# gwenzhang/GGA

Measured on AMD Instinct MI355X. Metric: kitti_frames_per_sec_gga_train_step, higher is better.
Workload: dtype f32 tensors; products on 2 x f16 operand planes (block-scaled), f32 accumulate - measured no less accurate than fp32 kernels: per convolution 0.7 x (dense) / 0.7-1.2 x (sparse) the RMS error of an fp32 FMA chain vs float64, whole-step losses over 8 seeds <= 2.5e-5 from float64 (fp32 CPU step: <= 1.6

## Files before the change

gga_amd/_lib.py:

```python
import ctypes as C
import os
import subprocess

_HERE = os.path.dirname(os.path.abspath(__file__))
LIB_PATH = os.path.join(_HERE, 'libgga_hip.so')
ABI_VERSION = 31

_lib = None

vp, i32, i64, f32, sz = C.c_void_p, C.c_int, C.c_int64, C.c_float, C.c_size_t
I3 = C.POINTER(C.c_int32 * 3)


class VoxelParams(C.Structure):
    _fields_ = [('voxel_size', C.c_float * 3), ('pc_range', C.c_float * 6),
                ('max_points', C.c_int32), ('max_voxels', C.c_int32)]


class PfnParams(C.Structure):
    _fields_ = [('voxel_size', C.c_float * 3), ('offsets', C.c_float * 3), ('eps', C.c_float),
                ('momentum', C.c_float), ('training', C.c_int32), ('in_features', C.c_int32),
                ('channels', C.c_int32)]


MAX_TASKS = 8


class Task(C.Structure):
    _fields_ = [('logits', vp), ('target', vp), ('n_heat', i64), ('focal_out', vp), ('focal_grad', vp), ('grad_logits', vp),
# ... 76 lines not shown
    'gga_dense_conv3x3_levels': (i32, [i32, vp, vp, vp, vp, i32, i32, i32, vp, i64, i32, vp, vp, vp, i32, i32, vp, vp]),
    'gga_dense_conv3x3_bn_bwd_pays': (i32, [i32, i32, i32, i32]),
    'gga_dense_conv3x3_bn_bwd_pays_planes': (i32, [i32, i32, i32, i32, i32]),
    'gga_dense_conv3x3_bn_bwd': (i32, [vp, vp, i32, i32, i32, i32, i32, vp, i64, i32, vp, i32, vp, vp, vp, i64, vp, vp, vp, vp, vp]),
    'gga_absmax_table_blocks': (i64, [i64]),
    'gga_absmax_table': (i32, [vp, i32, i64, vp, i32, vp]),
    'gga_pack_weights_table': (i32, [vp, i32, i64, i32, vp]),
    'gga_dense_wgrad3x3_block_amax': (i32, [vp, vp, i32, i32, i32, i32, i32, vp, i64, i64, i64, i64, i32, i32, vp, i32, vp, i32, vp, sz, vp]),
    'gga_dense_conv3x3_tile_rows': (i32, [i32, i32, i32, i32, i32]),
    'gga_dense_conv3x3_stat_rows': (i64, [i32, i32, i32, i32, i32, i32]),
    'gga_bn_stats_partials': (i32, [vp, vp, vp, vp, i64, i32, f32, f32, vp, vp, vp, i32, vp]),
    'gga_bn_stats_partials_cols': (i32, [vp, vp, vp, vp, i64, i32, f32, f32, vp, vp, vp, i32, i32, i32, vp]),
    'gga_bn_relu_workspace_bytes': (sz, [i64, i32]),
    'gga_bn_relu_mask_bytes': (sz, [i64, i32]),
    'gga_bn_relu_fwd_ex': (i32, [vp, vp, vp, vp, vp, vp, i64, i32, f32, f32, i32, i32, vp, i64, vp, vp, vp, i32, vp, vp, sz, vp]),
    'gga_bn_relu_bwd_ex': (i32, [vp, i64, vp, vp, vp, vp, i64, i32, i32, i32, vp, vp, vp, vp, vp, vp, sz, vp]),
    'gga_column_sums': (i32, [vp, i64, i32, vp, vp, sz, vp]),
    'gga_bn_relu_bwd_partials': (i32, [vp, i64, vp, vp, vp, i64, i32, i32, vp, i32, vp, vp, vp, vp, vp, sz, vp]),
    'gga_gn_relu_workspace_bytes': (sz, [i32, i32]),
    'gga_gn_relu_fwd': (i32, [vp, vp, vp, i32, i64, i32, i32, f32, i32, vp, vp, vp, vp, vp, sz, vp]),
    'gga_gn_relu_bwd': (i32, [vp, vp, vp, vp, vp, i32, i64, i32, i32, i32, vp, vp, vp, vp, vp, sz, vp]),
    'gga_bn_stats': (i32, [vp, vp, vp, vp, vp, i64, i32, f32, f32, i32, vp, vp, vp, sz, vp]),
    'gga_head_conv3x3_fwd': (i32, [vp, i64, vp, vp, vp, i32, i32, i32, i32, i32, vp, vp]),
    'gga_head_conv3x3_workspace_bytes': (sz, [i32]),
    'gga_head_conv3x3_wgrad': (i32, [vp, i64, vp, vp, i32, i32, i32, i32, i32, vp, vp, vp, sz, vp]),
    'gga_head_tail_bwd': (i32, [vp, vp, i64, vp, vp, vp, vp, i32, i32, i32, i32, i32, vp, i64, vp, vp, vp, vp, sz, vp]),
    'gga_head_tile_activity': (i32, [vp, i32, i32, i32, i32, vp, vp]),
    'gga_head_branch_bwd_workspace_bytes': (sz, [i32, i32, i32, i32]),
    'gga_head_branch_bwd': (i32, [vp, vp, i64, vp, vp, vp, vp, i32, i32, i32, i32, i32, vp, vp, vp, i64, vp, vp, vp, i32, vp, sz, vp]),
    'gga_heatmap_splat': (i32, [vp, i32, i32, i32, vp, i32, vp, vp, i32, vp]),
    'gga_focal_loss_workspace_bytes': (sz, [i64, i32]),
    'gga_focal_loss_fwd': (i32, [C.POINTER(TaskTable), f32, f32, f32, vp, sz, vp]),
    'gga_focal_loss_bwd': (i32, [C.POINTER(TaskTable), f32, f32, f32, vp]),
    'gga_gather_pred_fwd': (i32, [C.POINTER(TaskTable), i32, i32, i32, i32, vp]),
    'gga_gather_pred_bwd': (i32, [C.POINTER(TaskTable), i32, i32, i32, i32, vp]),
    'gga_box_losses_workspace_bytes': (sz, [i32, i32, i32]),
    'gga_box_losses_fwd': (i32, [C.POINTER(TaskTable), C.POINTER(LossParams), vp, sz, vp]),
    'gga_box_losses_bwd': (i32, [C.POINTER(TaskTable), i32, i32, vp]),
    'gga_box_iou_rotated': (i32, [vp, i32, vp, i32, i32, i32, vp, vp]),
    'gga_nms_rotated_workspace_bytes': (sz, [i32]),
    'gga_nms_rotated_sorted': (i32, [vp, i32, f32, i32, vp, vp, vp, sz, vp]),
    'gga_circle_nms_sorted': (i32, [vp, i32, C.c_double, i32, vp, vp, vp, sz, vp]),
    'gga_region_grow_workspace_bytes': (sz, [i64, i32]),
    'gga_region_grow': (i32, [vp, i64, i32, vp, vp, vp, i32, C.c_double, i32, vp, vp, sz, vp]),
    'gga_points_in_convex_polyhedra': (i32, [vp, i64, i32, vp, vp, i32, i32, vp, vp]),
    'gga_plane_inliers': (i32, [vp, i64, i32, vp, i32, C.c_double, vp, vp, vp]),
# ... 68 lines not shown
```

gga_amd/csrc/api.cc:

```cpp
#include <hip/hip_runtime.h>
#include <stdarg.h>
#include <stdio.h>

#include <mutex>
#include <vector>

#include "../../include/gga_hip.h"

static thread_local char g_err[512] = "";

void gga_set_error(const char* fmt, ...) {
    va_list ap;
    va_start(ap, fmt);
    vsnprintf(g_err, sizeof(g_err), fmt, ap);
    va_end(ap);
}

extern "C" const char* gga_last_error(void) { return g_err; }
extern "C" int gga_abi_version(void) { return 31; }

struct TimingSite {
    std::vector<hipEvent_t> ev;
    int cap = 0, count = 0;
    int64_t key = 0;
};
static TimingSite g_sites[GGA_TIME_SITES];
static std::mutex g_timing_mu;

hipEvent_t* gga_timing_acquire(int site, int64_t key) {
    if (site < 0 || site >= GGA_TIME_SITES) return nullptr;
    TimingSite& s = g_sites[site];
    if (s.cap == 0) return nullptr;
    std::lock_guard<std::mutex> lk(g_timing_mu);
    if (s.count >= s.cap || (s.key != 0 && s.key != key)) return nullptr;
    return &s.ev[2 * (size_t)s.count++];
}

extern "C" int gga_timing_begin(int site, int max_samples, int64_t key) {
    if (site < 0 || site >= GGA_TIME_SITES || max_samples < 0 || max_samples > 65536) {
        gga_set_error("gga_timing_begin: site %d / max_samples %d out of range", site, max_samples);
        return GGA_ERR_INVALID_ARG;
    }
// ... 36 lines not shown
```

gga_amd/csrc/headconv.hip:

```cpp
#include "gga_common.h"

#define HC_CIN 64
#define HC_MAXCO 4

#define HM_TW 32
#define HM_HW (HM_TW + 2)
#define HP_TR 13
#define HP_HR (HP_TR + 2)
#define HP_NPIX (HP_HR * HM_HW)
#define HP_NGRP 16
static_assert((HP_NPIX + 31) / 32 == HP_NGRP, "tile geometry");

template <int COUT, bool AFF>
__global__ __launch_bounds__(512, 4) void headconv_fwd16_kernel(const float* __restrict__ x, const float* __restrict__ w,
                                                            const float* __restrict__ bias, int B, int H, int W,
                                                            int tiles_x, int tiles_y, int n_tiles, int cout_total, int co_base,
                                                            const float* __restrict__ in_ss, int64_t xs, float* __restrict__ y) {
    typedef float f4 __attribute__((ext_vector_type(4)));
    typedef float f2 __attribute__((ext_vector_type(2)));
    constexpr int NT = COUT == 1 ? 1 : 2;
    constexpr int ZS = (9 * COUT) | 1;
    __shared__ float zt[HP_NGRP * 32 * ZS];
    __shared__ __attribute__((aligned(16))) float wl[16 * NT * 64];
    __shared__ __attribute__((aligned(16))) float ssl[4 * HC_CIN];
    __shared__ float bl[HC_MAXCO];
    const int per_img = tiles_x * tiles_y;
    const int lane = threadIdx.x & 63, wave = threadIdx.x >> 6;
    const int n = lane & 15, hq = lane >> 4;
    for (int i = threadIdx.x; i < 16 * NT * 64; i += 512) {
        const int e = i & 3, nn = (i >> 2) & 15, t = (i >> 6) % NT, jh = i / (64 * NT);
        const int c = 16 * (jh >> 2) + 4 * (jh & 3) + e, col = 16 * t + nn;
        const bool used = col < 9 * COUT;
        const int off = used ? col / COUT : 0, co = used ? col - off * COUT : 0;
        wl[i] = used ? w[((int64_t)(co_base + co) * HC_CIN + c) * 9 + off] : 0.0f;
    }
    if (AFF && threadIdx.x < 4 * HC_CIN) ssl[threadIdx.x] = threadIdx.x < 2 * HC_CIN ? in_ss[threadIdx.x] : 0.0f;
    if (threadIdx.x < COUT) bl[threadIdx.x] = bias ? bias[co_base + threadIdx.x] : 0.0f;
    __syncthreads();
    int loff[2][2], hrc[2][2];
#pragma unroll
// ... 36 lines not shown
                    const f2 hi = __builtin_elementwise_fma(f2{v[s][2], v[s][3]}, f2{sc[2], sc[3]}, f2{sf[2], sf[3]}); \
                    v[s] = f4{fmaxf(lo[0], 0.0f), fmaxf(lo[1], 0.0f), fmaxf(hi[0], 0.0f), fmaxf(hi[1], 0.0f)};       \
                }                                                                                                     \
            } else {                                                                                                  \
                _Pragma("unroll") for (int s = 0; s < 2; ++s) {                                                       \
                    const bool ok = (okm[U] >> s) & 1u;                                                               \
                    _Pragma("unroll") for (int e = 0; e < 4; ++e) v[s][e] = ok ? v[s][e] : 0.0f;                      \
                }                                                                                                     \
            }                                                                                                         \
            _Pragma("unroll") for (int e = 0; e < 4; ++e)                                                             \
                _Pragma("unroll") for (int t = 0; t < NT; ++t) {                                                      \
                    HQ_MFMA_(acc[0][t], v[0][e], bc[t][e]) HQ_MFMA_(acc[1][t], v[1][e], bc[t][e])                     \
                }                                                                                                     \
        }                                                                                                             \
        _Pragma("unroll") for (int s = 0; s < 2; ++s) _Pragma("unroll") for (int t = 0; t < NT; ++t)                  \
            if (16 * t + n < 9 * COUT) {                                                                              \
                float* zg = zt + ((wave + 8 * (U)) * 32 + 16 * s + 4 * hq) * ZS + 16 * t + n;                         \
                _Pragma("unroll") for (int v_ = 0; v_ < 4; ++v_) zg[v_ * ZS] = acc[s][t][v_];                         \
            } }
#define HQ_MFMA_(ACC, A, Bv) ACC = __builtin_amdgcn_mfma_f32_16x16x4f32(A, Bv, ACC, 0, 0, 0);
    const int xcd = blockIdx.x & 7, wg = blockIdx.x >> 3, wgs = ((int)gridDim.x + 7 - xcd) >> 3;
    const int chunk = (n_tiles + 7) >> 3;
    const int t_end = min(n_tiles, (xcd + 1) * chunk);
    int tile = xcd * chunk + wg;
    if (tile >= t_end) return;
    HQ_LOAD(tile, true, 0)
    HQ_LOAD(tile, true, 1)
    for (; tile < t_end; tile += wgs) {
        const int b = tile / per_img;
        const int rem = tile - b * per_img;
        const int y0 = (rem / tiles_x) * HP_TR, x0 = (rem % tiles_x) * HM_TW;
        const int nxt = tile + wgs;
        HQ_MMA(0)
        HQ_LOAD(nxt, nxt < t_end, 0)
        HQ_MMA(1)
        HQ_LOAD(nxt, nxt < t_end, 1)
        __syncthreads();
        if (threadIdx.x < HP_TR * HM_TW) {
            const int ty = threadIdx.x / HM_TW, tx = threadIdx.x - ty * HM_TW;
            const int oy = y0 + ty, ox = x0 + tx;
            if (oy < H && ox < W) {
                float s[COUT];
#pragma unroll
                for (int co = 0; co < COUT; ++co) s[co] = bl[co];
#pragma unroll
                for (int ky = 0; ky < 3; ++ky)
#pragma unroll
                    for (int kx = 0; kx < 3; ++kx) {
                        const float* z = zt + ((ty + ky) * HM_HW + tx + kx) * ZS + (ky * 3 + kx) * COUT;
#pragma unroll
                        for (int co = 0; co < COUT; ++co) s[co] += z[co];
                    }
                float* yo = y + (((int64_t)b * cout_total + co_base) * H + oy) * W + ox;
#pragma unroll
                for (int co = 0; co < COUT; ++co) yo[(int64_t)co * H * W] = s[co];
// ... 13 lines not shown
#define HG_PR (HG_TR + 2)
#define HG_PC (HG_TW + 2)
#define HG_GP (HG_PR * HG_PC)

__global__ __launch_bounds__(256) void head_tile_activity_kernel(const float* __restrict__ gy, int cout, int H, int W, int tiles_x,
                                                                 int tiles_y, int64_t n_tiles, uint8_t* __restrict__ act) {
    const int64_t t = (int64_t)blockIdx.x * 4 + (threadIdx.x >> 6);
    if (t >= n_tiles) return;
    const int lane = threadIdx.x & 63;
    const int per_img = tiles_x * tiles_y;
    const int b = (int)(t / per_img), rem = (int)(t - (int64_t)b * per_img);
    const int y0 = (rem / tiles_x) * HG_TR, x0 = (rem % tiles_x) * HG_TW;
    const int ya = max(y0 - 1, 0), yb = min(y0 + HG_TR, H - 1), xa = max(x0 - 1, 0), xb = min(x0 + HG_TW, W - 1);
    const int nc = xb - xa + 1, per_ch = (yb - ya + 1) * nc;
    uint32_t bits = 0;
    for (int i = lane; i < cout * per_ch; i += 64) {
        const int c = i / per_ch, q = i - c * per_ch;
        const int r = q / nc, col = q - r * nc;
        bits |= __float_as_uint(gy[(((int64_t)b * cout + c) * H + ya + r) * W + xa + col]);
    }
    const bool any = __ballot(bits != 0) != 0;
    if (lane == 0) act[t] = any ? 1 : 0;
}

struct HeadTileWalk {
    const uint8_t* act;
    int64_t base, stride, n_tiles;
    unsigned long long mask;
    __device__ __forceinline__ unsigned long long window(int64_t from) const {
        const int64_t t = from + (int64_t)(threadIdx.x & 63) * stride;
        return __ballot(t < n_tiles && act[t] != 0);
    }
    __device__ __forceinline__ HeadTileWalk(const uint8_t* a, int64_t first, int64_t s, int64_t n) : act(a), base(first), stride(s), n_tiles(n) {
        mask = window(base);
    }
    __device__ __forceinline__ int64_t next() {
        while (mask == 0) {
            if (base + 64 * stride >= n_tiles) return n_tiles;
            base += 64 * stride;
            mask = window(base);
        }
        const int k = __builtin_ctzll(mask);
        mask &= mask - 1;
        return base + k * stride;
    }
};

template <int COUT, bool AFF, bool MAP>
__global__ __launch_bounds__(512, 4) void headconv_wgrad16_kernel(const float* __restrict__ x, const float* __restrict__ dy,
                                                              int B, int H, int W, int tiles_x, int tiles_y, int n_tiles,
                                                              int cout_total, int co_base, const float* __restrict__ in_ss,
                                                              int64_t xs, const uint8_t* __restrict__ act,
                                                              float* __restrict__ partials) {
    typedef float f4 __attribute__((ext_vector_type(4)));
    typedef float f2 __attribute__((ext_vector_type(2)));
    constexpr int NT = COUT == 1 ? 1 : 2;
    constexpr int GN = (COUT * HG_GP + 511) / 512;
    __shared__ float gds[2][(COUT + 1) * HG_GP];
    __shared__ float red[HC_CIN * 33];
    __shared__ float bred[GN * 512];
    const int tid = threadIdx.x, lane = tid & 63, wave = tid >> 6;
    const int n = lane & 15, hq = lane >> 4;
    const int per_img = tiles_x * tiles_y;
    int gb[NT];
#pragma unroll
    for (int t = 0; t < NT; ++t) {
        const int col = n + 16 * t;
        const bool used = col < 9 * COUT;
        const int off = used ? col / COUT : 4, co = used ? col - off * COUT : COUT;
// ... 153 lines not shown
                "%s: specialised for %d input channels and 1..%d output channels (got %d -> %d)", fn, HC_CIN, HC_MAXCO,
                cin, cout);
    return GGA_OK;
}

extern "C" size_t gga_head_conv3x3_workspace_bytes(int cout) {
    return (size_t)HC_BLOCKS * ((size_t)cout * HC_CIN * 9 + cout) * sizeof(float);
}

static int headconv_stride(const char* fn, const void* x, int64_t xs) {
    GGA_REQUIRE(xs >= HC_CIN && xs % 4 == 0 && ((uintptr_t)x & 15) == 0,
                "%s: pixel stride %lld must be a multiple of 4 floats >= %d and the base 16-byte aligned", fn, (long long)xs, HC_CIN);
    return GGA_OK;
}

static int headconv_limits(const char* fn, int H, int W, int64_t xs, int rows, int64_t n_tiles) {
    GGA_REQUIRE(H < 16384 && W < 16384, "%s: height and width must be below 16384 (got H=%d W=%d)", fn, H, W);
    GGA_REQUIRE((int64_t)rows * W * xs < 2147483647ll,
                "%s: %d * W * pixel stride must be below 2^31 elements (got W=%d, pixel stride %lld)", fn, rows, W, (long long)xs);
    GGA_REQUIRE(n_tiles < 2147483647ll, "%s: too many tiles (%lld)", fn, (long long)n_tiles);
    return GGA_OK;
}

extern "C" int gga_head_conv3x3_fwd(const float* x, int64_t x_pixel_stride, const float* in_scale_shift, const float* weight,
                                    const float* bias, int B, int H, int W, int cin, int cout, float* y, void* stream_) {
    hipStream_t stream = (hipStream_t)stream_;
    if (int rc = headconv_check("gga_head_conv3x3_fwd", B, H, W, cin, cout)) return rc;
    GGA_REQUIRE(x && weight && y, "gga_head_conv3x3_fwd: null pointer argument");
    if (int rc = headconv_stride("gga_head_conv3x3_fwd", x, x_pixel_stride)) return rc;
    const int tx = (W + HM_TW - 1) / HM_TW, ty = (H + HP_TR - 1) / HP_TR;
    const int64_t n_tiles = (int64_t)B * tx * ty;
    if (int rc = headconv_limits("gga_head_conv3x3_fwd", H, W, x_pixel_stride, HP_HR + 1, n_tiles)) return rc;
    const dim3 grid((unsigned)(n_tiles < HC_BLOCKS ? n_tiles : HC_BLOCKS)), block(512);
#define HC_G(CO, BASE, AF) hipLaunchKernelGGL((headconv_fwd16_kernel<CO, AF>), grid, block, 0, stream, x, weight, bias, B, H, W, tx, ty, (int)n_tiles, cout, BASE, in_scale_shift, x_pixel_stride, y)
#define HC_F(CO, BASE) { if (in_scale_shift) HC_G(CO, BASE, true); else HC_G(CO, BASE, false); }
    switch (cout) {
        case 1: HC_F(1, 0); break;
        case 2: HC_F(2, 0); break;
        case 3: HC_F(3, 0); break;
        default: HC_F(2, 0); HC_F(2, 2); break;
    }
#undef HC_F
#undef HC_G
    GGA_CHECK_LAUNCH("headconv_fwd16_kernel");
    return GGA_OK;
}

static int headconv_wgrad_run(const char* fn, const float* x, int64_t x_pixel_stride, const float* in_scale_shift,
                              const float* grad_y, int B, int H, int W, int cin, int cout, float* grad_weight, float* grad_bias,
                              void* workspace, size_t workspace_bytes, const uint8_t* tile_act, hipStream_t stream) {
    if (int rc = headconv_check(fn, B, H, W, cin, cout)) return rc;
    if (int rc = headconv_stride(fn, x, x_pixel_stride)) return rc;
    GGA_REQUIRE(x && grad_y && grad_weight && workspace, "%s: null pointer argument", fn);
    const int tx = (W + HG_TW - 1) / HG_TW, ty = (H + HG_TR - 1) / HG_TR;
    const int64_t n_tiles = (int64_t)B * tx * ty;
    if (int rc = headconv_limits(fn, H, W, x_pixel_stride, HG_TR, n_tiles)) return rc;
    if (workspace_bytes < gga_head_conv3x3_workspace_bytes(cout)) {
        gga_set_error("%s: workspace too small", fn);
        return GGA_ERR_WORKSPACE;
    }
    const int nb = (int)(n_tiles < HC_BLOCKS ? n_tiles : HC_BLOCKS);
    float* partials = (float*)workspace;
#define HC_G(CO, BASE, AF, MP) hipLaunchKernelGGL((headconv_wgrad16_kernel<CO, AF, MP>), dim3(nb), dim3(512), 0, stream, x, grad_y, B, H, W, tx, ty, (int)n_tiles, cout, BASE, in_scale_shift, x_pixel_stride, tile_act, partials)
#define HC_A(CO, BASE, AF) { if (tile_act) HC_G(CO, BASE, AF, true); else HC_G(CO, BASE, AF, false); }
#define HC_W(CO, BASE) { if (in_scale_shift) HC_A(CO, BASE, true) else HC_A(CO, BASE, false) }
    switch (cout) {
        case 1: HC_W(1, 0); break;
// ... 329 lines not shown
```

gga_amd/dense_heads.py:

```python
import copy

import numpy as np
import os

import torch
from torch import nn

from . import dense_conv
from . import functional as F
from . import ops
from .cnn import ConvModule, build_conv_layer, kaiming_init
from .registry import HEADS, build_bbox_coder, build_head, build_loss

SRL_PRIORS = ((1.35, 0.48), (3.60, 0.68), (2.40, 0.28))


def multi_apply(func, *args, **kwargs):
    from functools import partial
    pfunc = partial(func, **kwargs) if kwargs else func
    return tuple(map(list, zip(*map(pfunc, *args))))


@HEADS.register_module()
class SeparateHead(nn.Module):
    def __init__(self, in_channels, heads, head_conv=64, final_kernel=1, init_bias=-2.19,
                 conv_cfg=dict(type='Conv2d'), norm_cfg=dict(type='BN2d'), bias='auto', init_cfg=None, **kwargs):
        assert init_cfg is None, 'To prevent abnormal initialization behavior, init_cfg is not allowed to be set'
        super().__init__()
        self.heads = heads
        self.init_bias = init_bias
        for head in self.heads:
            classes, num_conv = self.heads[head]
            conv_layers = []
            c_in = in_channels
            for _ in range(num_conv - 1):
                conv_layers.append(ConvModule(c_in, head_conv, kernel_size=final_kernel, stride=1,
                                              padding=final_kernel // 2, bias=bias, conv_cfg=conv_cfg,
# ... 76 lines not shown
        self.bbox_coder = build_bbox_coder(bbox_coder) if bbox_coder is not None else None
        self.num_anchor_per_locs = [n for n in num_classes]
        self.fp16_enabled = False
        self.pal_backprop = pal_backprop

        self.shared_conv = ConvModule(in_channels, share_conv_channel, kernel_size=3, padding=1,
                                      conv_cfg=conv_cfg, norm_cfg=norm_cfg, bias=bias)
        self.task_heads = nn.ModuleList()
        separate_head = dict(separate_head)
        for num_cls in num_classes:
            heads = copy.deepcopy(common_heads)
            heads.update(dict(heatmap=(num_cls, num_heatmap_convs)))
            separate_head.update(in_channels=share_conv_channel, heads=heads, num_cls=num_cls)
            self.task_heads.append(build_head(separate_head))
        self.with_velocity = 'vel' in common_heads.keys()
        assert not self.with_velocity, 'GGA does not support velocity (head:600-601)'
        assert self.norm_bbox, 'the HIP loss path implements norm_bbox=True (log-dims), as every GGA config uses'
        for name in ('loss_cls', 'loss_bbox'):
            red = getattr(getattr(self, name), 'reduction', 'mean')
            if red != 'mean':
                raise NotImplementedError(f"CenterHead_GGA: {name}.reduction={red!r}; the HIP loss path implements "
                                          f"reduction='mean' (configs/gga/gga_kitti_config.py:59-60)")

    def forward_single(self, x):
        x = self.shared_conv(x)
        branches, keys = [], []
        for ti, task in enumerate(self.task_heads):
            for head in getattr(task, 'heads', ()):
                mods = list(getattr(task, head))
                if (isinstance(task, SeparateHead) and len(mods) == 2 and isinstance(mods[0], ConvModule) and mods[0].with_norm
                        and mods[0].with_activation and isinstance(mods[0].norm, nn.modules.batchnorm._BatchNorm)
                        and isinstance(mods[0].activate, nn.ReLU)):
                    branches.append((mods[0].conv, mods[0].norm, mods[1]))
                    keys.append((ti, head))
        n_all = sum(len(getattr(task, 'heads', ())) for task in self.task_heads)
        outs = (F.head_branches(x, branches, sparse_grad=[head != 'heatmap' for _, head in keys])
                if branches and len(branches) == n_all and self.training else None)
        if outs is None:
            return [task(x) for task in self.task_heads]
        ret = [dict() for _ in self.task_heads]
        for (ti, head), y in zip(keys, outs):
            ret[ti][head] = y
        return ret

    def forward(self, feats):
        return multi_apply(self.forward_single, feats)

    def _feature_map_size(self):
        g = self.train_cfg['grid_size']
        osf = self.train_cfg['out_size_factor']
        return int(g[0]) // int(osf), int(g[1]) // int(osf)

    def draw_srl(self, batch_size):
        out = np.zeros((batch_size, len(self.task_heads)), np.float32)
        for b in range(batch_size):
            for t in range(len(self.task_heads)):
                mu, sd = SRL_PRIORS[t] if t < 2 else SRL_PRIORS[2]
                r = torch.normal(torch.tensor(mu), torch.tensor(sd))
                out[b, t] = float(torch.clamp(r, min=1e-3))
        return out

    def pack_targets(self, gt_labels_3d, GGA_boxes_img, GGA_lidar2img, GGA_init_pseudo_labels, GGA_bdry_masks,
                     GGA_in_box_points, img_metas, srl=None):
        tc = self.train_cfg
        B, T = len(gt_labels_3d), len(self.task_heads)
        K = int(tc['max_objs']) * int(tc['dense_reg'])
        osf = tc['out_size_factor']
        fw, fh = self._feature_map_size()
        vs = np.asarray(tc['voxel_size'], np.float32).astype(np.float64)
# ... 290 lines not shown
```

gga_amd/detectors.py:

```python
from collections import OrderedDict

import torch
from torch import nn

from .registry import (DETECTORS, build_backbone, build_head, build_middle_encoder, build_neck,
                       build_voxel_encoder)
from .voxel_layer import Voxelization


def _sub(cfg, key):
    if cfg is None:
        return None
    return cfg[key] if isinstance(cfg, dict) else getattr(cfg, key)


class PreparedInputs:

    def __init__(self, voxels, num_points, coors, n_frames):
        self.voxels, self.num_points, self.coors, self.n_frames = voxels, num_points, coors, n_frames

    def __len__(self):
        return self.n_frames

    def tensors(self):
        yield from (t for t in (self.voxels, self.num_points, self.coors) if t is not None)
        for extra in (getattr(self.coors, 'num_valid', None),):
            if extra is not None:
# ... 104 lines not shown
        if self.dynamic_voxelization:
            if self.front_reads_counts:
                coors.voxel_map.host_counts()
            return PreparedInputs(voxels, None, coors, len(points))
        if hasattr(self.pts_middle_encoder, 'build_indices'):
            coors = self.pts_middle_encoder.build_indices(coors, len(points))
        return PreparedInputs(voxels, num_points, coors, len(points))

    def forward_train(self, points=None, img_metas=None, gt_bboxes_3d=None, gt_labels_3d=None,
                      GGA_boxes_img=None, GGA_lidar2img=None, GGA_init_pseudo_labels=None, GGA_bdry_masks=None,
                      GGA_in_box_points=None, gt_labels=None, gt_bboxes=None, img=None, proposals=None,
                      gt_bboxes_ignore=None):
        img_feats, pts_feats = self.extract_feat(points, img=img, img_metas=img_metas)
        losses = dict()
        if pts_feats:
            losses.update(self.forward_pts_train(pts_feats, gt_bboxes_3d, gt_labels_3d, GGA_boxes_img,
                                                 GGA_lidar2img, GGA_init_pseudo_labels, GGA_bdry_masks,
                                                 GGA_in_box_points, img_metas, gt_bboxes_ignore))
        return losses

    def forward_pts_train(self, pts_feats, gt_bboxes_3d, gt_labels_3d, GGA_boxes_img, GGA_lidar2img,
                          GGA_init_pseudo_labels, GGA_bdry_masks, GGA_in_box_points, img_metas,
                          gt_bboxes_ignore=None):
        outs = self.pts_bbox_head(pts_feats)
        return self.pts_bbox_head.loss(gt_bboxes_3d, gt_labels_3d, outs, GGA_boxes_img, GGA_lidar2img,
                                       GGA_init_pseudo_labels, GGA_bdry_masks, GGA_in_box_points, img_metas)

    def forward(self, return_loss=True, **kwargs):
        if return_loss:
            return self.forward_train(**kwargs)
        return self.forward_test(**kwargs)

    def forward_test(self, points, img_metas, img=None, **kwargs):
        for var, name in [(points, 'points'), (img_metas, 'img_metas')]:
            if not isinstance(var, list):
                raise TypeError(f'{name} must be a list, but got {type(var)}')
        if len(points) != len(img_metas):
            raise ValueError(f'num of augmentations ({len(points)}) != num of image meta ({len(img_metas)})')
        if len(points) == 1:
            return self.simple_test(points[0], img_metas[0], None if img is None else img[0], **kwargs)
        raise NotImplementedError('test-time augmentation is not on the GGA path')

    @torch.no_grad()
    def simple_test_pts(self, x, img_metas, rescale=False):
        from .box3d import bbox3d2result
        outs = self.pts_bbox_head(x)
        bbox_list = self.pts_bbox_head.get_bboxes(outs, img_metas, rescale=rescale)
# ... 45 lines not shown
```

gga_amd/functional.py:

```python
import ctypes as C

import numpy as np
import torch

from . import _lib
from ._lib import LossParams, PfnParams, VoxelParams, check
import contextlib
import os

_DEFERRED_COUNTERS = None


def count_batch(bn):
    if _DEFERRED_COUNTERS is not None:
        _DEFERRED_COUNTERS.append(bn.num_batches_tracked)
    else:
        bn.num_batches_tracked += 1


@contextlib.contextmanager
def deferred_batch_counters():
    global _DEFERRED_COUNTERS
    prev, _DEFERRED_COUNTERS = _DEFERRED_COUNTERS, []
    try:
# ... 965 lines not shown
          and bn.momentum is not None and bn.training and torch.is_grad_enabled() and conv.out_channels <= 4
          and conv.kernel_size == (3, 3) and conv.stride == (1, 1) and conv.padding == (1, 1)
          and conv.dilation == (1, 1) and conv.groups == 1 and conv.padding_mode == 'zeros')
    if not ok:
        return head_conv3x3(bn_act(x, bn, relu=True), conv)
    count_batch(bn)
    partials = bn_partials_of(x)
    return _BnReluHeadConv3x3.apply(x, bn.weight, bn.bias, bn.running_mean, bn.running_var, conv.weight, conv.bias,
                                    float(bn.eps), float(bn.momentum), True, partials, sparse_grad)


_BRANCH_STREAMS = {}
HEAD_STREAMS = int(os.environ.get('GGA_HEAD_STREAMS', '2'))


def _branch_streams(device, n):
    k = max(1, min(HEAD_STREAMS, n))
    pool = _BRANCH_STREAMS.setdefault(device, [])
    while len(pool) < k - 1:
        pool.append(torch.cuda.Stream(device=device))
    return [torch.cuda.current_stream(device)] + pool[:k - 1]


class _HeadBranches(torch.autograd.Function):

    @staticmethod
    def forward(ctx, x, n, cfg, *t):
        from . import dense_conv
        w1, gam, bet, rm, rv, w2, b2 = (t[i * n:(i + 1) * n] for i in range(7))
        L = _lib.lib()
        B, C, H, W = x.shape
        rows, dev, tot = B * H * W, x.device, C * n
        tr = dense_conv._transposed(H, W)
        Y = torch.empty((B, tot, H, W), dtype=torch.float32, device=dev, memory_format=torch.channels_last)
        outs, saved_all, ss_all = [], [], []
        x_amax = dense_conv.tensor_amax(x) if dense_conv.PLANES == 2 else None
        pair_stats = {}
        for i in range(0, n - 1, 2):
            _, st = dense_conv._run(x, [w1[i].detach(), w1[i + 1].detach()], False, True, x_amax, None, Y, C * i)
            pair_stats[i], pair_stats[i + 1] = (st, 0), (st, C)
        all_stats = []
        for i in range(n):
            if i in pair_stats:
                all_stats.append(pair_stats[i])
            else:
                all_stats.append((dense_conv._run(x, w1[i].detach(), False, True, x_amax, None, Y, C * i)[1], 0))
        w2c = [w.contiguous() for w in w2]
        for i in range(n):
            outs.append(torch.empty((B, w2[i].shape[0], H, W), dtype=torch.float32, device=dev))
            saved_all.append(torch.empty(2 * C, dtype=torch.float32, device=dev))
            ss_all.append(torch.empty(2 * C, dtype=torch.float32, device=dev))
        streams = _branch_streams(dev, n)
        for st_ in streams[1:]:
            st_.wait_stream(streams[0])
        for i in range(n):
            eps, momentum = cfg[i][:2]
            stats, col = all_stats[i]
            tiles = int(stats.shape[0])
            with torch.cuda.stream(streams[i % len(streams)]):
                check(L.gga_bn_stats_partials_cols(_p(gam[i]), _p(bet[i]), _p(rm[i]), _p(rv[i]), rows, C, eps, momentum,
                                                   _p(saved_all[i]), _p(ss_all[i]), _p(stats), tiles, int(stats.shape[2]), col,
                                                   _stream()), 'gga_bn_stats_partials_cols')
                check(L.gga_head_conv3x3_fwd(Y.data_ptr() + 4 * C * i, tot, _p(ss_all[i]), _p(w2c[i]), _p(b2[i]), B, H, W, C,
                                             w2[i].shape[0], _p(outs[i]), _stream()), 'gga_head_conv3x3_fwd')
        for st_ in streams[1:]:
            streams[0].wait_stream(st_)
        ctx.save_for_backward(x, Y, *w1, *gam, *w2, *saved_all, *ss_all)
        ctx.n, ctx.has_bias, ctx.x_amax = n, [b is not None for b in b2], x_amax
        ctx.sparse_grad = [int(c[2]) for c in cfg]
        ctx.bn_src = dense_conv.bn_source(x, C) if dense_conv.BN_BWD_FUSED else None
        return tuple(outs)

    @staticmethod
    def backward(ctx, *gys):
        from . import dense_conv
        n = ctx.n
        t = ctx.saved_tensors
        x, Y = t[0], t[1]
        w1, gam, w2, saved_all, ss_all = (t[2 + i * n:2 + (i + 1) * n] for i in range(5))
        L = _lib.lib()
        B, C, H, W = x.shape
        rows, dev, tot = B * H * W, x.device, C * n
        G = torch.empty_like(Y)
        g_blocks = dense_conv.new_amax(dev, n)
        gw2, gb2, ggam, gbet = [], [], [], []
        gyc = [g.contiguous() for g in gys]
        w2c = [w.contiguous() for w in w2]
# ... 1 lines not shown
            gw2.append(torch.empty_like(w2c[i]))
            gb2.append(torch.empty(w2[i].shape[0], dtype=torch.float32, device=dev) if ctx.has_bias[i] else None)
            ggam.append(torch.empty(C, dtype=torch.float32, device=dev))
            gbet.append(torch.empty(C, dtype=torch.float32, device=dev))
        streams = _branch_streams(dev, n)
        for st_ in streams[1:]:
            st_.wait_stream(streams[0])
        for i in range(n):
            cout = w2[i].shape[0]
            with torch.cuda.stream(streams[i % len(streams)]):
                ws = _workspace('headbranch', L.gga_head_branch_bwd_workspace_bytes(B, H, W, cout), dev)
                check(L.gga_head_branch_bwd(_p(gyc[i]), Y.data_ptr() + 4 * C * i, tot, _p(ss_all[i]), _p(gam[i]), _p(saved_all[i]),
                                            _p(w2c[i]), B, H, W, C, cout, _p(gw2[i]), _p(gb2[i]), G.data_ptr() + 4 * C * i, tot,
                                            _p(ggam[i]), _p(gbet[i]), _p(g_blocks[i:i + 1] if g_blocks is not None else None),
                                            ctx.sparse_grad[i], _p(ws), ws.numel(), _stream()), 'gga_head_branch_bwd')
        for st_ in streams[1:]:
            streams[0].wait_stream(st_)
        wcat = [w.detach() for w in w1]
        g_amax = g_blocks.max().reshape(1) if g_blocks is not None else None
        gx = dense_conv.run_bn_bwd(G, wcat, g_amax, None, ctx.bn_src) if ctx.needs_input_grad[0] else None
        gwcat = dense_conv._wgrad(x, G, wcat, ctx.x_amax if dense_conv.PLANES == 2 else None, g_blocks, g_per_block=True)
        gw1 = list(gwcat.split(C, dim=0))
        none = [None] * n
        return (gx, None, None, *gw1, *ggam, *gbet, *none, *none, *gw2, *gb2)


def head_branches(x, branches, sparse_grad=None):
    from . import dense_conv
    rc = _rows_channels(x) if (x.is_cuda and x.dtype == torch.float32 and x.dim() == 4) else None
    if rc is None or x.shape[1] != 64 or not torch.is_grad_enabled() or not dense_conv.ENABLED or not dense_conv.WGRAD:
        return None
    for conv1, bn, conv2 in branches:
        ok = (dense_conv.eligible(conv1, x) and conv1.bias is None and conv1.out_channels == 64 and bn.affine
              and bn.track_running_stats and bn.momentum is not None and bn.training and conv2.out_channels <= 4
              and type(conv2) is torch.nn.Conv2d and conv2.in_channels == 64 and conv2.kernel_size == (3, 3)
              and conv2.stride == (1, 1) and conv2.padding == (1, 1) and conv2.dilation == (1, 1) and conv2.groups == 1
              and conv2.padding_mode == 'zeros')
        if not ok:
            return None
    for _, bn, _ in branches:
        count_batch(bn)
    n = len(branches)
    sparse = [True] * n if sparse_grad is None else [bool(s) for s in sparse_grad]
    assert len(sparse) == n
    cfg = tuple((float(bn.eps), float(bn.momentum), s) for (_, bn, _), s in zip(branches, sparse))
    cols = ([c1.weight for c1, _, _ in branches], [bn.weight for _, bn, _ in branches], [bn.bias for _, bn, _ in branches],
            [bn.running_mean for _, bn, _ in branches], [bn.running_var for _, bn, _ in branches],
            [c2.weight for _, _, c2 in branches], [c2.bias for _, _, c2 in branches])
    return _HeadBranches.apply(x, n, cfg, *[t for col in cols for t in col])


def head_conv3x3(x, conv):
    ok = (x.is_cuda and x.dtype == torch.float32 and x.dim() == 4 and x.shape[1] == 64
          and x.is_contiguous(memory_format=torch.channels_last) and conv.out_channels <= 4
          and conv.kernel_size == (3, 3) and conv.stride == (1, 1) and conv.padding == (1, 1)
          and conv.dilation == (1, 1) and conv.groups == 1 and conv.padding_mode == 'zeros')
    if not ok:
        return conv(x)
    return _HeadConv3x3.apply(x, conv.weight, conv.bias)


def centerpoint_detect(boxes, scores, labels, coder_range, coder_score_threshold, score_threshold, limit_range, nms_threshold,
                       pre_max_size, post_max_size, num_classes):
    _need_cuda(boxes, scores, labels)
    T, B, K, D = boxes.shape
    dev = boxes.device
    boxes, scores, labels = boxes.float().contiguous(), scores.float().contiguous(), labels.float().contiguous()
    out_boxes = torch.empty((B, T * K, D), dtype=torch.float32, device=dev)
    out_scores = torch.empty((B, T * K), dtype=torch.float32, device=dev)
    out_labels = torch.empty((B, T * K), dtype=torch.int32, device=dev)
    count = torch.zeros((B,), dtype=torch.int32, device=dev)
    offs, flag = [], 0
# ... 15 lines not shown
```

include/gga_hip.h:

```cpp
#ifndef GGA_HIP_H_
#define GGA_HIP_H_

#include <stddef.h>
#include <stdint.h>

#ifdef __cplusplus
extern "C" {
#endif

typedef enum {
    GGA_OK = 0,
    GGA_ERR_INVALID_ARG = -1,
    GGA_ERR_WORKSPACE = -2,
    GGA_ERR_LAUNCH = -3
} gga_status;

const char* gga_last_error(void);
int gga_abi_version(void);

enum {
    GGA_TIME_SCATTER_FWD = 0,
    GGA_TIME_DENSE_CONV = 1,
    GGA_TIME_SPARSE_CONV = 2,
    GGA_TIME_SPARSE_WGRAD = 3,
// ... 222 lines not shown
                    void* stream);
int gga_bn_relu_bwd_partials(const float* grad_masked, int64_t grad_row_stride, const float* x, const float* gamma,
                             const float* saved, int64_t rows, int channels, int training, const double* partials,
                             int n_partials, float* grad_x, float* grad_gamma, float* grad_beta, uint32_t* amax_grad_x,
                             void* workspace, size_t workspace_bytes, void* stream);

size_t gga_gn_relu_workspace_bytes(int B, int channels);
int gga_gn_relu_fwd(const float* x, const float* gamma, const float* beta, int B, int64_t rows_per_sample, int channels,
                    int groups, float eps, int relu, float* y, float* stat, float* scale_shift, uint32_t* amax_y,
                    void* workspace, size_t workspace_bytes, void* stream);
int gga_gn_relu_bwd(const float* grad_y, const float* x, const float* gamma, const float* stat, const float* scale_shift,
                    int B, int64_t rows_per_sample, int channels, int groups, int relu, float* grad_x, float* grad_gamma,
                    float* grad_beta, uint32_t* amax_grad_x, void* workspace, size_t workspace_bytes, void* stream);

int gga_bn_stats_partials(const float* gamma, const float* beta, float* running_mean, float* running_var,
                          int64_t rows, int channels, float eps, float momentum, float* saved, float* scale_shift,
                          const double* partials, int n_partials, void* stream);
int gga_bn_stats_partials_cols(const float* gamma, const float* beta, float* running_mean, float* running_var, int64_t rows,
                               int channels, float eps, float momentum, float* saved, float* scale_shift, const double* partials,
                               int n_partials, int partials_width, int column_offset, void* stream);

int gga_head_conv3x3_fwd(const float* x, int64_t x_pixel_stride, const float* in_scale_shift, const float* weight,
                         const float* bias, int B, int H, int W, int cin, int cout, float* y, void* stream);
size_t gga_head_conv3x3_workspace_bytes(int cout);
int gga_head_conv3x3_wgrad(const float* x, int64_t x_pixel_stride, const float* in_scale_shift, const float* grad_y,
                           int B, int H, int W, int cin, int cout, float* grad_weight, float* grad_bias,
                           void* workspace, size_t workspace_bytes, void* stream);

int gga_head_tail_bwd(const float* grad_y, const float* x, int64_t x_pixel_stride, const float* scale_shift,
                      const float* gamma, const float* saved, const float* weight, int B, int H, int W, int cin, int cout,
                      float* grad_x, int64_t grad_x_pixel_stride, float* grad_gamma, float* grad_beta, uint32_t* amax_grad_x,
                      void* workspace, size_t workspace_bytes, void* stream);

int gga_head_tile_activity(const float* grad_y, int B, int H, int W, int cout, uint8_t* tile_active, void* stream);

size_t gga_head_branch_bwd_workspace_bytes(int B, int H, int W, int cout);
int gga_head_branch_bwd(const float* grad_y, const float* x, int64_t x_pixel_stride, const float* scale_shift,
                        const float* gamma, const float* saved, const float* weight, int B, int H, int W, int cin, int cout,
                        float* grad_weight, float* grad_bias, float* grad_x, int64_t grad_x_pixel_stride, float* grad_gamma,
                        float* grad_beta, uint32_t* amax_grad_x, int sparse_grad_y, void* workspace, size_t workspace_bytes,
                        void* stream);

int gga_heatmap_splat(float* heatmap, int n_maps, int H, int W, const int32_t* objs, int n_obj,
                      const float* patch_table, const int32_t* patch_offsets, int max_radius,
                      void* stream);

// ... 149 lines not shown
```

Before: 525.4.

## Compute regression head forward convs only on tiles containing target cells

The training step now builds targets before the head forward and marks which 13x32 output tiles contain any target index for each task. The final 3x3 head conv for non-heatmap branches runs a tile-mapped kernel that skips inactive tiles and leaves zeros there, since only gathered cells feed the regression losses. This removes most of the dense forward conv work for regression branches. In exchange it adds a zero-fill of those outputs and a small marking kernel, and it makes the branch outputs valid only at target cells.

```diff
diff --git a/gga_amd/_lib.py b/gga_amd/_lib.py
--- a/gga_amd/_lib.py
+++ b/gga_amd/_lib.py
@@ -4,7 +4,7 @@
 
 _HERE = os.path.dirname(os.path.abspath(__file__))
 LIB_PATH = os.path.join(_HERE, 'libgga_hip.so')
-ABI_VERSION = 31
+ABI_VERSION = 32
 
 _lib = None
 
@@ -127,6 +127,9 @@
     'gga_gn_relu_bwd': (i32, [vp, vp, vp, vp, vp, i32, i64, i32, i32, i32, vp, vp, vp, vp, vp, sz, vp]),
     'gga_bn_stats': (i32, [vp, vp, vp, vp, vp, i64, i32, f32, f32, i32, vp, vp, vp, sz, vp]),
     'gga_head_conv3x3_fwd': (i32, [vp, i64, vp, vp, vp, i32, i32, i32, i32, i32, vp, vp]),
+    'gga_head_conv3x3_fwd_tiles': (i32, [vp, i64, vp, vp, vp, i32, i32, i32, i32, i32, vp, vp, vp]),
+    'gga_head_cell_tiles_count': (i64, [i32, i32, i32]),
+    'gga_head_cell_tiles': (i32, [vp, i32, i32, i32, i32, vp, vp]),
     'gga_head_conv3x3_workspace_bytes': (sz, [i32]),
     'gga_head_conv3x3_wgrad': (i32, [vp, i64, vp, vp, i32, i32, i32, i32, i32, vp, vp, vp, sz, vp]),
     'gga_head_tail_bwd': (i32, [vp, vp, i64, vp, vp, vp, vp, i32, i32, i32, i32, i32, vp, i64, vp, vp, vp, vp, sz, vp]),
diff --git a/gga_amd/csrc/api.cc b/gga_amd/csrc/api.cc
--- a/gga_amd/csrc/api.cc
+++ b/gga_amd/csrc/api.cc
@@ -17,7 +17,7 @@
 }
 
 extern "C" const char* gga_last_error(void) { return g_err; }
-extern "C" int gga_abi_version(void) { return 31; }
+extern "C" int gga_abi_version(void) { return 32; }
 
 struct TimingSite {
     std::vector<hipEvent_t> ev;
diff --git a/gga_amd/csrc/headconv.hip b/gga_amd/csrc/headconv.hip
--- a/gga_amd/csrc/headconv.hip
+++ b/gga_amd/csrc/headconv.hip
@@ -11,11 +11,51 @@
 #define HP_NGRP 16
 static_assert((HP_NPIX + 31) / 32 == HP_NGRP, "tile geometry");
 
-template <int COUT, bool AFF>
+struct HeadTileWalk {
+    const uint8_t* act;
+    int64_t base, stride, n_tiles;
+    unsigned long long mask;
+    __device__ __forceinline__ unsigned long long window(int64_t from) const {
+        const int64_t t = from + (int64_t)(threadIdx.x & 63) * stride;
+        return __ballot(t < n_tiles && act[t] != 0);
+    }
+    __device__ __forceinline__ HeadTileWalk(const uint8_t* a, int64_t first, int64_t s, int64_t n) : act(a), base(first), stride(s), n_tiles(n) {
+        mask = window(base);
+    }
+    __device__ __forceinline__ int64_t next() {
+        while (mask == 0) {
+            if (base + 64 * stride >= n_tiles) return n_tiles;
+            base += 64 * stride;
+            mask = window(base);
+        }
+        const int k = __builtin_ctzll(mask);
+        mask &= mask - 1;
+        return base + k * stride;
+    }
+};
+
+__global__ __launch_bounds__(256) void head_cell_tiles_kernel(const int64_t* __restrict__ ind, int64_t n, int K, int H, int W,
+                                                              int tiles_x, int tiles_y, uint8_t* __restrict__ act) {
+    const int64_t s = (int64_t)blockIdx.x * 256 + threadIdx.x;
+    if (s >= n) return;
+    const int64_t i = ind[s];
+    if (i < 0 || i >= (int64_t)H * W) return;
+    const int cy = (int)(i / W), cx = (int)(i - (int64_t)cy * W);
+    act[((s / K) * tiles_y + cy / HP_TR) * tiles_x + cx / HM_TW] = 1;
+}
+
+template <int COUT, bool AFF, bool MAP>
 __global__ __launch_bounds__(512, 4) void headconv_fwd16_kernel(const float* __restrict__ x, const float* __restrict__ w,
                                                             const float* __restrict__ bias, int B, int H, int W,
                                                             int tiles_x, int tiles_y, int n_tiles, int cout_total, int co_base,
-                                                            const float* __restrict__ in_ss, int64_t xs, float* __restrict__ y) {
+                                                            const float* __restrict__ in_ss, int64_t xs, float* __restrict__ y,
+                                                            const uint8_t* __restrict__ act) {
+    if (MAP) {
+        const int xcd_ = blockIdx.x & 7, chunk_ = (n_tiles + 7) >> 3;
+        const int end_ = min(n_tiles, (xcd_ + 1) * chunk_);
+        HeadTileWalk probe(act, xcd_ * chunk_ + ((int)blockIdx.x >> 3), ((int)gridDim.x + 7 - xcd_) >> 3, end_);
+        if (probe.next() >= end_) return;
+    }
     typedef float f4 __attribute__((ext_vector_type(4)));
     typedef float f2 __attribute__((ext_vector_type(2)));
     constexpr int NT = COUT == 1 ? 1 : 2;
@@ -98,15 +138,16 @@
     const int xcd = blockIdx.x & 7, wg = blockIdx.x >> 3, wgs = ((int)gridDim.x + 7 - xcd) >> 3;
     const int chunk = (n_tiles + 7) >> 3;
     const int t_end = min(n_tiles, (xcd + 1) * chunk);
-    int tile = xcd * chunk + wg;
+    HeadTileWalk walk(MAP ? act : nullptr, MAP ? xcd * chunk + wg : t_end, wgs, t_end);
+    int tile = MAP ? (int)walk.next() : xcd * chunk + wg;
     if (tile >= t_end) return;
     HQ_LOAD(tile, true, 0)
     HQ_LOAD(tile, true, 1)
-    for (; tile < t_end; tile += wgs) {
+    for (int nxt; tile < t_end; tile = nxt) {
         const int b = tile / per_img;
         const int rem = tile - b * per_img;
         const int y0 = (rem / tiles_x) * HP_TR, x0 = (rem % tiles_x) * HM_TW;
-        const int nxt = tile + wgs;
+        nxt = MAP ? (int)walk.next() : tile + wgs;
         HQ_MMA(0)
         HQ_LOAD(nxt, nxt < t_end, 0)
         HQ_MMA(1)
@@ -166,29 +207,6 @@
     const bool any = __ballot(bits != 0) != 0;
     if (lane == 0) act[t] = any ? 1 : 0;
 }
-
-struct HeadTileWalk {
-    const uint8_t* act;
-    int64_t base, stride, n_tiles;
-    unsigned long long mask;
-    __device__ __forceinline__ unsigned long long window(int64_t from) const {
-        const int64_t t = from + (int64_t)(threadIdx.x & 63) * stride;
-        return __ballot(t < n_tiles && act[t] != 0);
-    }
-    __device__ __forceinline__ HeadTileWalk(const uint8_t* a, int64_t first, int64_t s, int64_t n) : act(a), base(first), stride(s), n_tiles(n) {
-        mask = window(base);
-    }
-    __device__ __forceinline__ int64_t next() {
-        while (mask == 0) {
-            if (base + 64 * stride >= n_tiles) return n_tiles;
-            base += 64 * stride;
-            mask = window(base);
-        }
-        const int k = __builtin_ctzll(mask);
-        mask &= mask - 1;
-        return base + k * stride;
-    }
-};
 
 template <int COUT, bool AFF, bool MAP>
 __global__ __launch_bounds__(512, 4) void headconv_wgrad16_kernel(const float* __restrict__ x, const float* __restrict__ dy,
@@ -388,18 +406,20 @@
     return GGA_OK;
 }
 
-extern "C" int gga_head_conv3x3_fwd(const float* x, int64_t x_pixel_stride, const float* in_scale_shift, const float* weight,
-                                    const float* bias, int B, int H, int W, int cin, int cout, float* y, void* stream_) {
-    hipStream_t stream = (hipStream_t)stream_;
-    if (int rc = headconv_check("gga_head_conv3x3_fwd", B, H, W, cin, cout)) return rc;
-    GGA_REQUIRE(x && weight && y, "gga_head_conv3x3_fwd: null pointer argument");
-    if (int rc = headconv_stride("gga_head_conv3x3_fwd", x, x_pixel_stride)) return rc;
+static int headconv_fwd_run(const char* fn, const float* x, int64_t x_pixel_stride, const float* in_scale_shift, const float* weight,
+                            const float* bias, int B, int H, int W, int cin, int cout, const uint8_t* tile_act, bool tiled,
+                            float* y, hipStream_t stream) {
+    if (int rc = headconv_check(fn, B, H, W, cin, cout)) return rc;
+    GGA_REQUIRE(x && weight && y, "%s: null pointer argument", fn);
+    GGA_REQUIRE(!tiled || tile_act, "%s: null tile map", fn);
+    if (int rc = headconv_stride(fn, x, x_pixel_stride)) return rc;
     const int tx = (W + HM_TW - 1) / HM_TW, ty = (H + HP_TR - 1) / HP_TR;
     const int64_t n_tiles = (int64_t)B * tx * ty;
-    if (int rc = headconv_limits("gga_head_conv3x3_fwd", H, W, x_pixel_stride, HP_HR + 1, n_tiles)) return rc;
+    if (int rc = headconv_limits(fn, H, W, x_pixel_stride, HP_HR + 1, n_tiles)) return rc;
     const dim3 grid((unsigned)(n_tiles < HC_BLOCKS ? n_tiles : HC_BLOCKS)), block(512);
-#define HC_G(CO, BASE, AF) hipLaunchKernelGGL((headconv_fwd16_kernel<CO, AF>), grid, block, 0, stream, x, weight, bias, B, H, W, tx, ty, (int)n_tiles, cout, BASE, in_scale_shift, x_pixel_stride, y)
-#define HC_F(CO, BASE) { if (in_scale_shift) HC_G(CO, BASE, true); else HC_G(CO, BASE, false); }
+#define HC_G(CO, BASE, AF, MP) hipLaunchKernelGGL((headconv_fwd16_kernel<CO, AF, MP>), grid, block, 0, stream, x, weight, bias, B, H, W, tx, ty, (int)n_tiles, cout, BASE, in_scale_shift, x_pixel_stride, y, tile_act)
+#define HC_A(CO, BASE, AF) { if (tile_act) HC_G(CO, BASE, AF, true); else HC_G(CO, BASE, AF, false); }
+#define HC_F(CO, BASE) { if (in_scale_shift) HC_A(CO, BASE, true) else HC_A(CO, BASE, false) }
     switch (cout) {
         case 1: HC_F(1, 0); break;
         case 2: HC_F(2, 0); break;
@@ -407,8 +427,39 @@
         default: HC_F(2, 0); HC_F(2, 2); break;
     }
 #undef HC_F
+#undef HC_A
 #undef HC_G
     GGA_CHECK_LAUNCH("headconv_fwd16_kernel");
+    return GGA_OK;
+}
+
+extern "C" int gga_head_conv3x3_fwd(const float* x, int64_t x_pixel_stride, const float* in_scale_shift, const float* weight,
+                                    const float* bias, int B, int H, int W, int cin, int cout, float* y, void* stream) {
+    return headconv_fwd_run("gga_head_conv3x3_fwd", x, x_pixel_stride, in_scale_shift, weight, bias, B, H, W, cin, cout, nullptr, false,
+                            y, (hipStream_t)stream);
+}
+
+extern "C" int gga_head_conv3x3_fwd_tiles(const float* x, int64_t x_pixel_stride, const float* in_scale_shift, const float* weight,
+                                          const float* bias, int B, int H, int W, int cin, int cout, const uint8_t* tile_active,
+                                          float* y, void* stream) {
+    return headconv_fwd_run("gga_head_conv3x3_fwd_tiles", x, x_pixel_stride, in_scale_shift, weight, bias, B, H, W, cin, cout,
+                            tile_active, true, y, (hipStream_t)stream);
+}
+
+extern "C" int64_t gga_head_cell_tiles_count(int B, int H, int W) {
+    if (B < 1 || H < 1 || W < 1) return 0;
+    return (int64_t)B * ((H + HP_TR - 1) / HP_TR) * ((W + HM_TW - 1) / HM_TW);
+}
+
+extern "C" int gga_head_cell_tiles(const int64_t* ind, int n_maps, int K, int H, int W, uint8_t* tile_active, void* stream) {
+    GGA_REQUIRE(n_maps >= 1 && K >= 1 && H >= 1 && W >= 1, "gga_head_cell_tiles: bad sizes (n_maps=%d K=%d H=%d W=%d)", n_maps, K, H, W);
+    GGA_REQUIRE(ind, "gga_head_cell_tiles: null index pointer");
+    GGA_REQUIRE(tile_active, "gga_head_cell_tiles: null tile map");
+    const int64_t n = (int64_t)n_maps * K;
+    GGA_REQUIRE((n + 255) / 256 < 2147483647ll, "gga_head_cell_tiles: too many slots (%lld)", (long long)n);
+    hipLaunchKernelGGL(head_cell_tiles_kernel, dim3((unsigned)((n + 255) / 256)), dim3(256), 0, (hipStream_t)stream, ind, n, K, H, W,
+                       (W + HM_TW - 1) / HM_TW, (H + HP_TR - 1) / HP_TR, tile_active);
+    GGA_CHECK_LAUNCH("head_cell_tiles_kernel");
     return GGA_OK;
 }
 
diff --git a/gga_amd/dense_heads.py b/gga_amd/dense_heads.py
--- a/gga_amd/dense_heads.py
+++ b/gga_amd/dense_heads.py
@@ -13,6 +13,9 @@
 from .registry import HEADS, build_bbox_coder, build_head, build_loss
 
 SRL_PRIORS = ((1.35, 0.48), (3.60, 0.68), (2.40, 0.28))
+
+
+FWD_CELLS = os.environ.get('GGA_HEAD_FWD_CELLS', '1') != '0'
 
 
 def multi_apply(func, *args, **kwargs):
@@ -135,7 +138,7 @@
                 raise NotImplementedError(f"CenterHead_GGA: {name}.reduction={red!r}; the HIP loss path implements "
                                           f"reduction='mean' (configs/gga/gga_kitti_config.py:59-60)")
 
-    def forward_single(self, x):
+    def forward_single(self, x, cells=None):
         x = self.shared_conv(x)
         branches, keys = [], []
         for ti, task in enumerate(self.task_heads):
@@ -147,8 +150,17 @@
                     branches.append((mods[0].conv, mods[0].norm, mods[1]))
                     keys.append((ti, head))
         n_all = sum(len(getattr(task, 'heads', ())) for task in self.task_heads)
-        outs = (F.head_branches(x, branches, sparse_grad=[head != 'heatmap' for _, head in keys])
-                if branches and len(branches) == n_all and self.training else None)
+        fused = bool(branches) and len(branches) == n_all and self.training
+        tile_maps = None
+        if fused and cells is not None and x.is_cuda:
+            if len(cells) != len(self.task_heads):
+                raise ValueError(f'CenterHead_GGA: cells for {len(cells)} tasks, the head has {len(self.task_heads)}')
+            if any(c.shape[0] != x.shape[0] for c in cells):
+                raise ValueError('CenterHead_GGA: cells must be [B, K] per task, with the batch size of the feature map')
+            maps = F.head_cell_tiles(list(cells), x.shape[2], x.shape[3])
+            tile_maps = [None if head == 'heatmap' else maps[ti] for ti, head in keys]
+        outs = (F.head_branches(x, branches, sparse_grad=[head != 'heatmap' for _, head in keys], tile_maps=tile_maps)
+                if fused else None)
         if outs is None:
             return [task(x) for task in self.task_heads]
         ret = [dict() for _ in self.task_heads]
@@ -156,8 +168,10 @@
             ret[ti][head] = y
         return ret
 
-    def forward(self, feats):
-        return multi_apply(self.forward_single, feats)
+    def forward(self, feats, cells=None):
+        if cells is None:
+            return multi_apply(self.forward_single, feats)
+        return multi_apply(self.forward_single, feats, cells=cells)
 
     def _feature_map_size(self):
         g = self.train_cfg['grid_size']
diff --git a/gga_amd/detectors.py b/gga_amd/detectors.py
--- a/gga_amd/detectors.py
+++ b/gga_amd/detectors.py
@@ -3,6 +3,7 @@
 import torch
 from torch import nn
 
+from . import dense_heads
 from .registry import (DETECTORS, build_backbone, build_head, build_middle_encoder, build_neck,
                        build_voxel_encoder)
 from .voxel_layer import Voxelization
@@ -153,7 +154,13 @@
     def forward_pts_train(self, pts_feats, gt_bboxes_3d, gt_labels_3d, GGA_boxes_img, GGA_lidar2img,
                           GGA_init_pseudo_labels, GGA_bdry_masks, GGA_in_box_points, img_metas,
                           gt_bboxes_ignore=None):
-        outs = self.pts_bbox_head(pts_feats)
+        head = self.pts_bbox_head
+        if dense_heads.FWD_CELLS and isinstance(head, dense_heads.CenterHead_GGA):
+            targets = head.get_targets(gt_bboxes_3d, gt_labels_3d, GGA_boxes_img, GGA_lidar2img, GGA_init_pseudo_labels,
+                                       GGA_bdry_masks, GGA_in_box_points, img_metas, device=pts_feats[0].device)
+            outs = head(pts_feats, cells=targets[2])
+            return head.loss_from_targets(outs, *targets)
+        outs = head(pts_feats)
         return self.pts_bbox_head.loss(gt_bboxes_3d, gt_labels_3d, outs, GGA_boxes_img, GGA_lidar2img,
                                        GGA_init_pseudo_labels, GGA_bdry_masks, GGA_in_box_points, img_metas)
 
diff --git a/gga_amd/functional.py b/gga_amd/functional.py
--- a/gga_amd/functional.py
+++ b/gga_amd/functional.py
@@ -1011,12 +1011,29 @@
     return [torch.cuda.current_stream(device)] + pool[:k - 1]
 
 
+def head_cell_tiles(inds, H, W):
+    _need_cuda(*inds)
+    L = _lib.lib()
+    T = len(inds)
+    B, K = inds[0].shape
+    for ind in inds:
+        if ind.dtype != torch.int64 or tuple(ind.shape) != (B, K) or not ind.is_contiguous():
+            raise ValueError(f'head_cell_tiles: every ind must be a contiguous int64 [B, K] tensor (got {ind.dtype} {tuple(ind.shape)})')
+    per = int(L.gga_head_cell_tiles_count(B, H, W))
+    maps = torch.zeros((T, per), dtype=torch.uint8, device=inds[0].device)
+    one = all(inds[t].data_ptr() == inds[0].data_ptr() + 8 * B * K * t for t in range(T))
+    for t in range(1 if one else T):
+        check(L.gga_head_cell_tiles(_p(inds[t]), (T if one else 1) * B, K, H, W, _p(maps[t]), _stream()), 'gga_head_cell_tiles')
+    return list(maps.unbind(0))
+
+
 class _HeadBranches(torch.autograd.Function):
 
     @staticmethod
-    def forward(ctx, x, n, cfg, *t):
+    def forward(ctx, x, n, cfg, maps, *t):
         from . import dense_conv
         w1, gam, bet, rm, rv, w2, b2 = (t[i * n:(i + 1) * n] for i in range(7))
+        maps = [None] * n if maps is None else list(maps)
         L = _lib.lib()
         B, C, H, W = x.shape
         rows, dev, tot = B * H * W, x.device, C * n
@@ -1035,8 +1052,14 @@
             else:
                 all_stats.append((dense_conv._run(x, w1[i].detach(), False, True, x_amax, None, Y, C * i)[1], 0))
         w2c = [w.contiguous() for w in w2]
+        sizes = [B * w2[i].shape[0] * H * W if maps[i] is not None else 0 for i in range(n)]
+        tiled = torch.zeros(sum(sizes), dtype=torch.float32, device=dev) if any(sizes) else None
         for i in range(n):
-            outs.append(torch.empty((B, w2[i].shape[0], H, W), dtype=torch.float32, device=dev))
+            if maps[i] is not None:
+                o = sum(sizes[:i])
+                outs.append(tiled[o:o + sizes[i]].view(B, w2[i].shape[0], H, W))
+            else:
+                outs.append(torch.empty((B, w2[i].shape[0], H, W), dtype=torch.float32, device=dev))
             saved_all.append(torch.empty(2 * C, dtype=torch.float32, device=dev))
             ss_all.append(torch.empty(2 * C, dtype=torch.float32, device=dev))
         streams = _branch_streams(dev, n)
@@ -1050,8 +1073,13 @@
                 check(L.gga_bn_stats_partials_cols(_p(gam[i]), _p(bet[i]), _p(rm[i]), _p(rv[i]), rows, C, eps, momentum,
                                                    _p(saved_all[i]), _p(ss_all[i]), _p(stats), tiles, int(stats.shape[2]), col,
                                                    _stream()), 'gga_bn_stats_partials_cols')
-                check(L.gga_head_conv3x3_fwd(Y.data_ptr() + 4 * C * i, tot, _p(ss_all[i]), _p(w2c[i]), _p(b2[i]), B, H, W, C,
-                                             w2[i].shape[0], _p(outs[i]), _stream()), 'gga_head_conv3x3_fwd')
+                if maps[i] is not None:
+                    check(L.gga_head_conv3x3_fwd_tiles(Y.data_ptr() + 4 * C * i, tot, _p(ss_all[i]), _p(w2c[i]), _p(b2[i]), B, H, W,
+                                                       C, w2[i].shape[0], _p(maps[i]), _p(outs[i]), _stream()),
+                          'gga_head_conv3x3_fwd_tiles')
+                else:
+                    check(L.gga_head_conv3x3_fwd(Y.data_ptr() + 4 * C * i, tot, _p(ss_all[i]), _p(w2c[i]), _p(b2[i]), B, H, W, C,
+                                                 w2[i].shape[0], _p(outs[i]), _stream()), 'gga_head_conv3x3_fwd')
         for st_ in streams[1:]:
             streams[0].wait_stream(st_)
         ctx.save_for_backward(x, Y, *w1, *gam, *w2, *saved_all, *ss_all)
@@ -1099,10 +1127,10 @@
         gwcat = dense_conv._wgrad(x, G, wcat, ctx.x_amax if dense_conv.PLANES == 2 else None, g_blocks, g_per_block=True)
         gw1 = list(gwcat.split(C, dim=0))
         none = [None] * n
-        return (gx, None, None, *gw1, *ggam, *gbet, *none, *none, *gw2, *gb2)
-
-
-def head_branches(x, branches, sparse_grad=None):
+        return (gx, None, None, None, *gw1, *ggam, *gbet, *none, *none, *gw2, *gb2)
+
+
+def head_branches(x, branches, sparse_grad=None, tile_maps=None):
     from . import dense_conv
     rc = _rows_channels(x) if (x.is_cuda and x.dtype == torch.float32 and x.dim() == 4) else None
     if rc is None or x.shape[1] != 64 or not torch.is_grad_enabled() or not dense_conv.ENABLED or not dense_conv.WGRAD:
@@ -1124,7 +1152,15 @@
     cols = ([c1.weight for c1, _, _ in branches], [bn.weight for _, bn, _ in branches], [bn.bias for _, bn, _ in branches],
             [bn.running_mean for _, bn, _ in branches], [bn.running_var for _, bn, _ in branches],
             [c2.weight for _, _, c2 in branches], [c2.bias for _, _, c2 in branches])
-    return _HeadBranches.apply(x, n, cfg, *[t for col in cols for t in col])
+    if tile_maps is not None:
+        B, _, H, W = x.shape
+        per = int(_lib.lib().gga_head_cell_tiles_count(B, H, W))
+        assert len(tile_maps) == n
+        for m in tile_maps:
+            if m is not None and not (m.dtype == torch.uint8 and m.device == x.device and m.is_contiguous() and m.numel() == per):
+                raise ValueError(f'head_branches: a tile map must be a contiguous uint8 tensor of {per} tiles on {x.device}')
+        tile_maps = tuple(tile_maps) if any(m is not None for m in tile_maps) else None
+    return _HeadBranches.apply(x, n, cfg, tile_maps, *[t for col in cols for t in col])
 
 
 def head_conv3x3(x, conv):
diff --git a/include/gga_hip.h b/include/gga_hip.h
--- a/include/gga_hip.h
+++ b/include/gga_hip.h
@@ -268,6 +268,11 @@
 
 int gga_head_conv3x3_fwd(const float* x, int64_t x_pixel_stride, const float* in_scale_shift, const float* weight,
                          const float* bias, int B, int H, int W, int cin, int cout, float* y, void* stream);
+int gga_head_conv3x3_fwd_tiles(const float* x, int64_t x_pixel_stride, const float* in_scale_shift, const float* weight,
+                               const float* bias, int B, int H, int W, int cin, int cout, const uint8_t* tile_active, float* y,
+                               void* stream);
+int64_t gga_head_cell_tiles_count(int B, int H, int W);
+int gga_head_cell_tiles(const int64_t* ind, int n_maps, int K, int H, int W, uint8_t* tile_active, void* stream);
 size_t gga_head_conv3x3_workspace_bytes(int cout);
 int gga_head_conv3x3_wgrad(const float* x, int64_t x_pixel_stride, const float* in_scale_shift, const float* grad_y,
                            int B, int H, int W, int cin, int cout, float* grad_weight, float* grad_bias,
```

After: 534.2, median of 6. 1.02x the previous value.
